# bliunlpr/Robust_e2e_gan

Hardware: NVIDIA B200
Metric: utterances/sec (joint step fwd/bwd) (higher is better)
Workload: dtype fp32

## Files before the change

### robust_e2e_gan_b200/csrc/attloc_loop.cu

```cuda
#include <math_constants.h>

#include "attloc_common.cuh"
#include "tc_common.cuh"

namespace re2e {
namespace {

#ifdef RE2E_ATT_DEBUG
__device__ long long g_loop_dbg[2][16 * 512];
#define LOOP_DBG_DECL                                                  \
  __shared__ long long dbg_acc[16];                                    \
  if (threadIdx.x == 0)                                                \
    for (int i_ = 0; i_ < 16; ++i_) dbg_acc[i_] = 0;                   \
  long long dbg_last = clock64()
#define LOOP_MARK(slot)                                              \
  do {                                                               \
    if (threadIdx.x == 0) {                                          \
      const long long t_ = clock64();                                \
      dbg_acc[slot] += t_ - dbg_last;                                \
      dbg_last = t_;                                                 \
    }                                                                \
  } while (0)
#define LOOP_DBG_FLUSH(which)                                                                   \
  do {                                                                                          \
    if (threadIdx.x == 0)                                                                       \
      for (int i_ = 0; i_ < 16; ++i_) g_loop_dbg[which][blockIdx.x * 16 + i_] = dbg_acc[i_];    \
  } while (0)
#else
#define LOOP_DBG_DECL
#define LOOP_MARK(slot)
#define LOOP_DBG_FLUSH(which)
#endif

__device__ __forceinline__ void cp_async4(void *dst_smem, const void *src_gmem) {
  asm volatile("cp.async.ca.shared.global [%0], [%1], 4;" ::"r"(smem_u32(dst_smem)), "l"(src_gmem) : "memory");
}
__device__ __forceinline__ void cp_async_commit() { asm volatile("cp.async.commit_group;" ::: "memory"); }
__device__ __forceinline__ void cp_async_wait_all() { asm volatile("cp.async.wait_group 0;" ::: "memory"); }

__device__ __forceinline__ void warp_reduce10(float (&v)[10], int lane) {
  {
    const bool up = lane & 16;
#pragma unroll
    for (int i = 0; i < 5; ++i) {
      const float send = up ? v[i] : v[i + 5], keep = up ? v[i + 5] : v[i];
      v[i] = keep + __shfl_xor_sync(0xffffffffu, send, 16);
    }
  }
  {
    const bool up = lane & 8;
#pragma unroll
    for (int i = 0; i < 2; ++i) {
      const float send = up ? v[i] : v[i + 3], keep = up ? v[i + 3] : v[i];
// ... 11 lines not shown
    const bool up = lane & 2;
    const float send = up ? v[0] : v[2], keep = up ? v[2] : v[0];
    v[0] = keep + __shfl_xor_sync(0xffffffffu, send, 2);
  }
  v[0] += __shfl_xor_sync(0xffffffffu, v[0], 1);
}

constexpr int kLP = 8;
constexpr int kLW = 2 * kLP;
constexpr int kLT = kLW * 32;
constexpr int kLMaxCL = 8;
constexpr int kKG = 12;

struct LoopGeom {
  int tloc_max, App, CKp, Thp, Dp;
  int col_enc, ncols;
};

struct LoopFwdParams {
  const float *pre, *enc, *dec_proj, *att_init, *W_att, *W_conv, *gvec, *gvec_b;
  float scaling;
  float *c_all, *w_all, *conv_all;
  int S, B, Th, D, A, C, K;
  LoopGeom g;
};

struct LoopBwdParams {
  const float *pre, *enc, *dec_proj, *att_init, *w_all, *conv_all, *dc_all, *dw_all, *W_att, *W_conv, *gvec;
  float scaling;
  float *d_pre, *d_decproj, *acc_slots;
  int slot_stride;
  int S, B, Th, D, A, C, K;
  LoopGeom g;
};

template <int APL, int CP, int DPL>
__global__ void __launch_bounds__(kLT, 1) attloc_loop_fwd_kernel(const LoopFwdParams p) {
  constexpr int NT = kLT;
  constexpr int WP = CP + 1;
  constexpr int CPP = (CP + 3) & ~3;
  extern __shared__ __align__(128) unsigned char smraw[];
  const LoopGeom g = p.g;
  const int C = CP == 10 ? 10 : p.C;
  const int Th = p.Th, D = p.D, A = p.A, K = p.K, S = p.S, B = p.B, filts = (p.K - 1) / 2;
  const int tid = threadIdx.x, lane = tid & 31, warp = tid >> 5, half = warp & 1, pair = warp >> 1;
  const int CL = (int)cluster_nctarank(), rank = (int)cluster_ctarank();
  const int b = blockIdx.x / CL;
  const int t0 = min(Th, rank * g.tloc_max), t1 = min(Th, t0 + g.tloc_max), tloc = t1 - t0;
  const int nch = (tloc + kLP - 1) / kLP;
  const int Dp = g.Dp, Dh = (D + 1) / 2;

  uint64_t *full = reinterpret_cast<uint64_t *>(smraw);
  uint64_t *xbar = full + 1;
  uint64_t *tbar = xbar + 2;
  float *tile = reinterpret_cast<float *>(smraw + 128);
  float *app = tile + (size_t)g.tloc_max * (A + D);
  float *wc_s = app + g.App;
  float *watt_s = wc_s + g.CKp;
  float *convp = watt_s + A * WP;
  float *conv_s = convp + round4(kKQ * g.tloc_max * CP);
  float *e_all = conv_s + g.tloc_max * CPP;
  float *epart = e_all + 2 * g.Thp;
  float *cred = epart + round4(2 * g.tloc_max);
  float *cbuf = cred + kLP * Dp;

  const uint32_t xbytes = (uint32_t)Th * 4u + (rank == 0 ? (uint32_t)CL * (uint32_t)D * 4u : 0u);
  if (tid == 0) {
    mbar_init(full, 1);
    mbar_init(&xbar[0], 1);
    mbar_init(&xbar[1], 1);
    mbar_init(tbar, 1);
    mbar_fence_init();
    mbar_expect_tx(&xbar[0], xbytes);
    mbar_expect_tx(&xbar[1], xbytes);
    if (rank == 0) mbar_expect_tx(tbar, (uint32_t)CL * (uint32_t)D * 4u);
  }
  cluster_arrive_relaxed();
  float gv[APL];
#pragma unroll
  for (int j = 0; j < APL; ++j) gv[j] = __ldg(p.gvec + half * (A / 2) + lane + 32 * j);
  const float gb = __ldg(p.gvec_b);
  for (int i = tid; i < C * K; i += NT) wc_s[i] = __ldg(p.W_conv + i);
  for (int i = tid; i < A * C; i += NT) { const int a = i / C; watt_s[a * WP + (i - a * C)] = __ldg(p.W_att + i); }
  pdl_wait();
  if (tid == 0 && tloc > 0) {
    mbar_expect_tx(full, (uint32_t)tloc * (uint32_t)(A + D) * 4u);
    bulk_g2s(tile, p.pre + ((size_t)b * Th + t0) * A, (uint32_t)tloc * A * 4u, full);
    bulk_g2s(tile + (size_t)g.tloc_max * A, p.enc + ((size_t)b * Th + t0) * D, (uint32_t)tloc * D * 4u, full);
  }
  for (int i = tid; i < g.App; i += NT) {
    const int t = i - filts;
    app[i] = (t >= 0 && t < Th) ? __ldg(p.att_init + (size_t)b * Th + t) : 0.0f;
  }
  __syncthreads();
  constexpr int APH = (APL + 1) / 2;
  float2 WattP[APH][CP];
#pragma unroll
  for (int jp = 0; jp < APH; ++jp) {
    const int a0 = half * (A / 2) + lane + 32 * (2 * jp), a1 = a0 + 32;
#pragma unroll
    for (int c = 0; c < CP; ++c)
      WattP[jp][c] = make_float2(c < C ? watt_s[a0 * WP + c] : 0.0f, (c < C && 2 * jp + 1 < APL) ? watt_s[a1 * WP + c] : 0.0f);
  }
  uint32_t dmask = 0;
#pragma unroll
  for (int j = 0; j < DPL; ++j)
    if (lane + 32 * j < Dh && half * Dh + lane + 32 * j < D) dmask |= 1u << j;
  const int aoff = half * (A / 2) + lane;
  cluster_wait();
  if (tloc > 0) mbar_wait(full, 0);
  LOOP_DBG_DECL;
  LOOP_MARK(0);

  for (int s = 0; s < S; ++s) {
    const uint32_t par = (uint32_t)s & 1u, ph = ((uint32_t)s >> 1) & 1u;
    float *e_cur = e_all + par * g.Thp;
    float *cb = cbuf + par * kLMaxCL * Dp;
    float dp[APL];
#pragma unroll
    for (int j = 0; j < APL; ++j) dp[j] = __ldg(p.dec_proj + ((size_t)s * B + b) * A + aoff + 32 * j);

    {
      const int ntg = (tloc + kTG - 1) / kTG;
      const int Kq = (K + kKQ - 1) / kKQ;
      const int nitems = ntg * C * kKQ;
      for (int item = tid; item < nitems; item += NT) {
        const int tg = item % ntg, rest = item / ntg, c = rest % C, kq = rest / C;
        const int k0 = kq * Kq, k1 = min(K, k0 + Kq);
        const float *wr = wc_s + c * K;
        const float *ar = app + t0 + kTG * tg;
        float a0 = 0.f, a1 = 0.f, a2 = 0.f, a3 = 0.f, a4 = 0.f;
        float x0 = ar[k0], x1 = ar[k0 + 1], x2 = ar[k0 + 2], x3 = ar[k0 + 3];
// ... 16 lines not shown
    __syncthreads();
    LOOP_MARK(1);
    for (int i = tid; i < tloc * CPP; i += NT) {
      const int tl = i / CPP, c = i - tl * CPP;
      float v = 0.0f;
      if (c < C) {
#pragma unroll
        for (int kq = 0; kq < kKQ; ++kq) v += convp[((size_t)kq * g.tloc_max + tl) * CP + c];
        if (p.conv_all) p.conv_all[(((size_t)s * B + b) * Th + t0 + tl) * C + c] = v;
      }
      conv_s[i] = v;
    }
    __syncthreads();
    LOOP_MARK(2);

    float acc[DPL];
#pragma unroll
    for (int j = 0; j < DPL; ++j) acc[j] = 0.0f;
#pragma unroll 2
    for (int q = 0; q < nch; ++q) {
      const int tl = kLP * q + pair;
      if (tl < tloc) {
        const float *cvp = conv_s + tl * CPP;
        float cv[CPP];
#pragma unroll
        for (int c4 = 0; c4 < CPP; c4 += 4) {
          const float4 t4 = *reinterpret_cast<const float4 *>(cvp + c4);
          cv[c4] = t4.x; cv[c4 + 1] = t4.y; cv[c4 + 2] = t4.z; cv[c4 + 3] = t4.w;
        }
        const float *row = tile + (size_t)tl * A + aoff;
        const float pw = app[filts + t0 + tl];
        const float *er = tile + (size_t)g.tloc_max * A + (size_t)tl * D + half * Dh + lane;
        float part = 0.0f;
#pragma unroll
        for (int jp = 0; jp < APH; ++jp) {
          const bool two = 2 * jp + 1 < APL;
          float2 u = make_float2(dp[2 * jp] + row[64 * jp], two ? dp[2 * jp + 1] + row[64 * jp + 32] : 0.0f);
#pragma unroll
          for (int c = 0; c < CP; ++c) u = __ffma2_rn(WattP[jp][c], make_float2(cv[c], cv[c]), u);
          part = fmaf(gv[2 * jp], tanh_ex2(u.x), part);
          if (two) part = fmaf(gv[2 * jp + 1], tanh_ex2(u.y), part);
        }
#pragma unroll
        for (int j = 0; j < DPL; ++j)
          if (dmask & (1u << j)) acc[j] = fmaf(pw, er[32 * j], acc[j]);
        part = warp_sum(part);
        if (lane == 0) epart[2 * tl + half] = part;
      }
    }
#pragma unroll
    for (int j = 0; j < DPL; ++j)
      if (dmask & (1u << j)) cred[pair * Dp + half * Dh + lane + 32 * j] = acc[j];
    LOOP_MARK(3);
    __syncthreads();
    LOOP_MARK(4);

    for (int d = tid; d < D; d += NT) {
      float sum = 0.0f;
#pragma unroll
      for (int pr = 0; pr < kLP; ++pr) sum += cred[pr * Dp + d];
      st_async_f32(dsmem_addr(cb + rank * Dp + d, 0u), s > 0 ? sum : 0.0f, dsmem_addr(&xbar[par], 0u));
    }
    for (int i = tid; i < tloc * CL; i += NT) {
      const int r = i / tloc, tl = i - r * tloc;
      const float e = p.scaling * ((epart[2 * tl] + epart[2 * tl + 1]) + gb);
      st_async_f32(dsmem_addr(e_cur + t0 + tl, (uint32_t)r), e, dsmem_addr(&xbar[par], (uint32_t)r));
    }
    LOOP_MARK(5);
    mbar_wait(&xbar[par], ph);
    LOOP_MARK(6);
    float M = -CUDART_INF_F;
    for (int t = lane; t < Th; t += 32) M = fmaxf(M, e_cur[t]);
    M = warp_max(M);
    float Ssum = 0.0f;
    for (int t = lane; t < Th; t += 32) Ssum += __expf(e_cur[t] - M);
    Ssum = warp_sum(Ssum);
    const float inv = 1.0f / Ssum;
    for (int t = tid; t < Th; t += NT) {
      const float w = __expf(e_cur[t] - M) * inv;
      app[filts + t] = w;
      if (t >= t0 && t < t1) p.w_all[((size_t)s * B + b) * Th + t] = w;
    }
    if (rank == 0 && s > 0) {
      for (int d = tid; d < D; d += NT) {
        float sum = 0.0f;
        for (int r = 0; r < CL; ++r) sum += cb[r * Dp + d];
        p.c_all[((size_t)(s - 1) * B + b) * D + d] = sum;
      }
    }
    if (tid == 0) mbar_expect_tx(&xbar[par], xbytes);
    __syncthreads();
    LOOP_MARK(7);
  }
  {
    float acc[DPL];
#pragma unroll
    for (int j = 0; j < DPL; ++j) acc[j] = 0.0f;
    for (int q = 0; q < nch; ++q) {
      const int tl = kLP * q + pair;
      if (tl < tloc) {
        const float pw = app[filts + t0 + tl];
        const float *er = tile + (size_t)g.tloc_max * A + (size_t)tl * D + half * Dh + lane;
#pragma unroll
        for (int j = 0; j < DPL; ++j)
          if (dmask & (1u << j)) acc[j] = fmaf(pw, er[32 * j], acc[j]);
      }
    }
#pragma unroll
    for (int j = 0; j < DPL; ++j)
      if (dmask & (1u << j)) cred[pair * Dp + half * Dh + lane + 32 * j] = acc[j];
    __syncthreads();
    float *cb = cbuf + ((uint32_t)S & 1u) * kLMaxCL * Dp;
    for (int d = tid; d < D; d += NT) {
      float sum = 0.0f;
#pragma unroll
      for (int pr = 0; pr < kLP; ++pr) sum += cred[pr * Dp + d];
      st_async_f32(dsmem_addr(cb + rank * Dp + d, 0u), sum, dsmem_addr(tbar, 0u));
    }
    if (rank == 0) {
      mbar_wait(tbar, 0);
      for (int d = tid; d < D; d += NT) {
        float sum = 0.0f;
        for (int r = 0; r < CL; ++r) sum += cb[r * Dp + d];
        p.c_all[((size_t)(S - 1) * B + b) * D + d] = sum;
      }
    }
  }
  LOOP_DBG_FLUSH(0);
}

template <int N>
__device__ __forceinline__ void tmem_ldn(uint32_t taddr, float *v);
template <>
__device__ __forceinline__ void tmem_ldn<1>(uint32_t taddr, float *v) {
  uint32_t r0;
  asm volatile("tcgen05.ld.sync.aligned.32x32b.x1.b32 {%0}, [%1];" : "=r"(r0) : "r"(taddr));
  v[0] = __uint_as_float(r0);
}
template <>
__device__ __forceinline__ void tmem_ldn<2>(uint32_t taddr, float *v) {
  uint32_t r0, r1;
  asm volatile("tcgen05.ld.sync.aligned.32x32b.x2.b32 {%0, %1}, [%2];" : "=r"(r0), "=r"(r1) : "r"(taddr));
// ... 47 lines not shown
template <int N>
__device__ __forceinline__ void tmem_load(uint32_t taddr, float *v) {
  if constexpr (N >= 8) { tmem_ldn<8>(taddr, v); if constexpr (N > 8) tmem_load<N - 8>(taddr + 8, v + 8); }
  else if constexpr (N >= 4) { tmem_ldn<4>(taddr, v); if constexpr (N > 4) tmem_load<N - 4>(taddr + 4, v + 4); }
  else if constexpr (N >= 2) { tmem_ldn<2>(taddr, v); if constexpr (N > 2) tmem_load<N - 2>(taddr + 2, v + 2); }
  else { tmem_ldn<1>(taddr, v); }
}
template <int N>
__device__ __forceinline__ void tmem_store(uint32_t taddr, const float *v) {
  if constexpr (N >= 8) { tmem_stn<8>(taddr, v); if constexpr (N > 8) tmem_store<N - 8>(taddr + 8, v + 8); }
  else if constexpr (N >= 4) { tmem_stn<4>(taddr, v); if constexpr (N > 4) tmem_store<N - 4>(taddr + 4, v + 4); }
  else if constexpr (N >= 2) { tmem_stn<2>(taddr, v); if constexpr (N > 2) tmem_store<N - 2>(taddr + 2, v + 2); }
  else { tmem_stn<1>(taddr, v); }
}

template <int APL, int CP, int DPL2>
__global__ void __launch_bounds__(kLT, 1) attloc_loop_bwd_kernel(const LoopBwdParams p) {
  constexpr int NT = kLT;
  constexpr int WP = CP + 1;
  constexpr int CPP = (CP + 3) & ~3;
  constexpr int CH2 = (CP + 1) / 2;
  extern __shared__ __align__(128) unsigned char smraw[];
  const LoopGeom g = p.g;
  const int C = CP == 10 ? 10 : p.C;
  const int Th = p.Th, D = p.D, A = p.A, K = p.K, S = p.S, B = p.B, filts = (p.K - 1) / 2;
  const int tid = threadIdx.x, lane = tid & 31, warp = tid >> 5, half = warp & 1, pair = warp >> 1;
  const int CL = (int)cluster_nctarank(), rank = (int)cluster_ctarank();
  const int b = blockIdx.x / CL;
  const int t0 = min(Th, rank * g.tloc_max), t1 = min(Th, t0 + g.tloc_max), tloc = t1 - t0;
  const int nchx = (tloc + kLP - 1) / kLP;
  const int nche = (tloc + kLW - 1) / kLW;
  const int nchx_max = (g.tloc_max + kLP - 1) / kLP, nche_max = (g.tloc_max + kLW - 1) / kLW;

  uint64_t *done_x = reinterpret_cast<uint64_t *>(smraw);
  uint64_t *xbar1 = done_x + 1;
  uint64_t *xbar2 = xbar1 + 2;
  uint32_t *tmem_slot = reinterpret_cast<uint32_t *>(xbar2 + 2);
  float *xs = reinterpret_cast<float *>(smraw + 128);
  float *dcvT = xs + (size_t)g.tloc_max * A;
  float *app = dcvT + 2 * CP * g.App;
  float *wc_s = app + g.App;
  float *conv_s = wc_s + g.CKp;
  float *w_s = conv_s + g.tloc_max * CPP;
  float *dwt_s = w_s + round4(g.tloc_max);
  float *de_s = dwt_s + round4(g.tloc_max);
  float *dwn_s = de_s + round4(g.tloc_max);
  float *dcv_p = dwn_s + round4(g.tloc_max);
  float *ddp_w = dcv_p + 2 * g.tloc_max * 16;
  float *scr = ddp_w + kLW * (A / 2);
  float *ddp_x = scr + max(A * WP, round4(kKQ * CP * g.tloc_max));
  float *xch = ddp_x + 2 * kLMaxCL * A;
  float *slot = p.acc_slots + (size_t)blockIdx.x * p.slot_stride;

  const uint32_t x1bytes = (uint32_t)CL * 4u;
  const uint32_t x2bytes = (uint32_t)Th * (uint32_t)C * 4u + (rank == 0 ? (uint32_t)CL * (uint32_t)A * 4u : 0u);
  if (tid == 0) {
    mbar_init(done_x, kLW);
    for (int i = 0; i < 2; ++i) { mbar_init(&xbar1[i], 1); mbar_init(&xbar2[i], 1); }
    mbar_fence_init();
    for (int i = 0; i < 2; ++i) { mbar_expect_tx(&xbar1[i], x1bytes); mbar_expect_tx(&xbar2[i], x2bytes); }
  }
  cluster_arrive_relaxed();
  if (warp == 0) tmem_alloc(tmem_slot, 512);
  float gv[APL];
#pragma unroll
  for (int j = 0; j < APL; ++j) gv[j] = __ldg(p.gvec + half * (A / 2) + lane + 32 * j);
  for (int i = tid; i < C * K; i += NT) wc_s[i] = __ldg(p.W_conv + i);
  for (int i = tid; i < A * C; i += NT) { const int a = i / C; scr[a * WP + (i - a * C)] = __ldg(p.W_att + i); }
  {
    const int padn = g.App - Th;
    for (int i = tid; i < 2 * CP * padn; i += NT) {
      const int c = i / padn, o = i - c * padn;
      dcvT[c * g.App + (o < filts ? o : Th + o)] = 0.0f;
    }
    for (int i = tid; i < g.tloc_max * CPP; i += NT) conv_s[i] = 0.0f;
    for (int i = tid; i < round4(g.tloc_max); i += NT) dwn_s[i] = 0.0f;
  }
  tc_fence_before();
  __syncthreads();
  tc_fence_after();
  const uint32_t tbase = *tmem_slot + ((uint32_t)(32 * (warp & 3)) << 16);
  const uint32_t tcol_pre = tbase + (uint32_t)((warp >> 2) * nchx_max * APL);
  const uint32_t tcol_enc = tbase + (uint32_t)(g.col_enc + (warp >> 2) * nche_max * DPL2);
  float2 WattC[APL][CH2];
#pragma unroll
  for (int j = 0; j < APL; ++j) {
    const int a = half * (A / 2) + lane + 32 * j;
#pragma unroll
    for (int c2 = 0; c2 < CH2; ++c2)
      WattC[j][c2] = make_float2(2 * c2 < C ? scr[a * WP + 2 * c2] : 0.0f, 2 * c2 + 1 < C ? scr[a * WP + 2 * c2 + 1] : 0.0f);
  }
  const int aoff = half * (A / 2) + lane;
  pdl_wait();
  for (int q = 0; q < nchx; ++q) {
    const int tl = kLP * q + pair;
    float v[APL];
#pragma unroll
    for (int j = 0; j < APL; ++j) v[j] = tl < tloc ? __ldg(p.pre + ((size_t)b * Th + t0 + tl) * A + aoff + 32 * j) : 0.0f;
    tmem_store<APL>(tcol_pre + (uint32_t)(q * APL), v);
  }
  for (int q = 0; q < nche; ++q) {
    const int tl = kLW * q + warp;
    float v[DPL2];
#pragma unroll
    for (int j = 0; j < DPL2; ++j)
      v[j] = (tl < tloc && lane + 32 * j < D) ? __ldg(p.enc + ((size_t)b * Th + t0 + tl) * D + lane + 32 * j) : 0.0f;
    tmem_store<DPL2>(tcol_enc + (uint32_t)(q * DPL2), v);
  }
  tmem_wait_st();
  __syncthreads();
  cluster_wait();

  float pacc[kKG];
#pragma unroll
  for (int i = 0; i < kKG; ++i) pacc[i] = 0.0f;
  float dgv[APL];
#pragma unroll
  for (int j = 0; j < APL; ++j) dgv[j] = 0.0f;
  float dgb = 0.0f;
  const int nkg = (K + kKG - 1) / kKG;
  const bool conv_thread = tid >= A && tid - A < C * nkg;
  const int cw_c = conv_thread ? (tid - A) / nkg : 0, cw_kb = conv_thread ? ((tid - A) % nkg) * kKG : 0;
  LOOP_DBG_DECL;
  LOOP_MARK(0);

  for (int it = 0; it < S; ++it) {
    const int s = S - 1 - it;
    const uint32_t par = (uint32_t)it & 1u, ph = ((uint32_t)it >> 1) & 1u;
    float *dcv_cur = dcvT + par * CP * g.App;
    float *ddpx = ddp_x + par * kLMaxCL * A;
    float *xc = xch + par * kLMaxCL;
    const size_t sb = (size_t)s * B + b;
    float dcr[DPL2];
#pragma unroll
    for (int j = 0; j < DPL2; ++j) dcr[j] = (p.dc_all && lane + 32 * j < D) ? __ldg(p.dc_all + sb * D + lane + 32 * j) : 0.0f;
    float dp[APL];
#pragma unroll
    for (int j = 0; j < APL; ++j) dp[j] = __ldg(p.dec_proj + sb * A + aoff + 32 * j);
    for (int i = tid; i < tloc; i += NT) {
      w_s[i] = __ldg(p.w_all + sb * Th + t0 + i);
      dwt_s[i] = dwn_s[i] + (p.dw_all ? __ldg(p.dw_all + sb * Th + t0 + i) : 0.0f);
    }
    for (int i = tid; i < tloc * C; i += NT) {
      const int tl = i / C;
      conv_s[tl * CPP + (i - tl * C)] = __ldg(p.conv_all + (sb * Th + t0) * C + i);
    }
    {
      const float *prev = s == 0 ? p.att_init + (size_t)b * Th : p.w_all + (sb - B) * Th;
      for (int i = tid; i < g.App; i += NT) {
        const int t = i - filts;
        app[i] = (t >= 0 && t < Th) ? __ldg(prev + t) : 0.0f;
      }
    }
    __syncthreads();
    LOOP_MARK(1);

    for (int q = 0; q < nche; ++q) {
      const int tl = kLW * q + warp;
      float ev[DPL2];
      tmem_load<DPL2>(tcol_enc + (uint32_t)(q * DPL2), ev);
      tmem_wait_ld();
      float dot = 0.0f;
#pragma unroll
      for (int j = 0; j < DPL2; ++j) dot = fmaf(dcr[j], ev[j], dot);
      dot = warp_sum(dot);
      if (lane == 0 && tl < tloc) dwt_s[tl] += dot;
    }
    __syncthreads();
    LOOP_MARK(2);
    if (warp == 0) {
      float s1 = 0.0f;
      for (int tl = lane; tl < tloc; tl += 32) s1 = fmaf(w_s[tl], dwt_s[tl], s1);
      s1 = warp_sum(s1);
      if (lane < CL) st_async_f32(dsmem_addr(xc + rank, (uint32_t)lane), s1, dsmem_addr(&xbar1[par], (uint32_t)lane));
    }
    mbar_wait(&xbar1[par], ph);
    float Stot = 0.0f;
    for (int r = 0; r < CL; ++r) Stot += xc[r];
    for (int tl = tid; tl < tloc; tl += NT) de_s[tl] = p.scaling * w_s[tl] * (dwt_s[tl] - Stot);
    if (tid == 0) {
      mbar_expect_tx(&xbar1[par], x1bytes);
// ... 87 lines not shown
    for (int j = 0; j < APL; ++j) ddp_w[warp * (A / 2) + lane + 32 * j] = ddp[j];
    __syncthreads();
    LOOP_MARK(5);

    for (int item = tid; item < tloc * C; item += NT) {
      const int c = item / tloc, tl = item - c * tloc;
      const float v = dcv_p[tl * 16 + c] + dcv_p[(g.tloc_max + tl) * 16 + c];
      for (int r = 0; r < CL; ++r)
        st_async_f32(dsmem_addr(dcv_cur + c * g.App + filts + t0 + tl, (uint32_t)r), v, dsmem_addr(&xbar2[par], (uint32_t)r));
    }
    for (int a = tid; a < A; a += NT) {
      const int h = a >= A / 2 ? 1 : 0, ai = a - h * (A / 2);
      float sd = 0.0f;
#pragma unroll
      for (int pr = 0; pr < kLP; ++pr) sd += ddp_w[(2 * pr + h) * (A / 2) + ai];
      st_async_f32(dsmem_addr(ddpx + rank * A + a, 0u), sd, dsmem_addr(&xbar2[par], 0u));
    }
    if (warp == kLW - 1) {
      float s2 = 0.0f;
      for (int tl = lane; tl < tloc; tl += 32) s2 += de_s[tl];
      dgb += warp_sum(s2);
    }
    LOOP_MARK(6);
    if (tid < A) {
#pragma unroll 5
      for (int tl = 0; tl < tloc; ++tl) {
        const float dt = xs[(size_t)tl * A + tid];
#pragma unroll
        for (int c4 = 0; c4 < CPP; c4 += 4) {
          const float4 t4 = *reinterpret_cast<const float4 *>(conv_s + tl * CPP + c4);
          if (c4 < CP) pacc[c4] = fmaf(dt, t4.x, pacc[c4]);
// ... 8 lines not shown
#pragma unroll
      for (int i = 0; i < kKG - 1; ++i) x[i] = ar[t0 + i];
#pragma unroll 12
      for (int tl = 0; tl < tloc; ++tl) {
        x[kKG - 1] = ar[t0 + tl + kKG - 1];
        const float dv = dcv_p[tl * 16 + cw_c] + dcv_p[(g.tloc_max + tl) * 16 + cw_c];
#pragma unroll
        for (int i = 0; i < kKG; ++i) pacc[i] = fmaf(dv, x[i], pacc[i]);
#pragma unroll
        for (int i = 0; i < kKG - 1; ++i) x[i] = x[i + 1];
      }
    }
    LOOP_MARK(7);
    mbar_wait(&xbar2[par], ph);
    LOOP_MARK(8);
    if (rank == 0) {
      for (int a = tid; a < A; a += NT) {
        float sd = 0.0f;
        for (int r = 0; r < CL; ++r) sd += ddpx[r * A + a];
        p.d_decproj[sb * A + a] = sd;
      }
    }
    if (s > 0) {
      const int nsg = (tloc + kTG - 1) / kTG;
      const int Kq = (K + kKQ - 1) / kKQ;
      const int nitems = nsg * C * kKQ;
      for (int item = tid; item < nitems; item += NT) {
        const int sg = item % nsg, rest = item / nsg, c = rest % C, kq = rest / C;
        const int k0 = kq * Kq, k1 = min(K, k0 + Kq);
        const float *wr = wc_s + c * K;
        const float *dr = dcv_cur + c * g.App + (t0 + kTG * sg) + 2 * filts;
        float a0 = 0.f, a1 = 0.f, a2 = 0.f, a3 = 0.f, a4 = 0.f;
        float x1 = dr[1 - k0], x2 = dr[2 - k0], x3 = dr[3 - k0], x4 = dr[4 - k0];
#pragma unroll 5
        for (int k = k0; k < k1; ++k) {
          const float x0 = dr[-k], wv = wr[k];
// ... 63 lines not shown
inline int pick_cl(int B, int Th) {
  const int sms = num_sms();
  int CL = 1;
  while (CL < kLMaxCL && B * CL * 2 <= sms) CL *= 2;
  while (CL > 1 && (Th + CL - 1) / CL < kLP) CL /= 2;
  return CL;
}

inline void loop_geom_common(int Th, int D, int C, int K, int CL, LoopGeom &g) {
  const int filts = (K - 1) / 2;
  g.tloc_max = (Th + CL - 1) / CL;
  g.App = round4(Th + 2 * filts + 8);
  g.CKp = round4(C * K);
  g.Thp = round4(Th);
  g.Dp = round4(D);
  g.col_enc = 0;
  g.ncols = 0;
}

inline bool loop_geom_fwd(int B, int Th, int D, int A, int C, int K, int CP, int &CL, LoopGeom &g, size_t &smem) {
  CL = pick_cl(B, Th);
  const int CPP = round4(CP);
  for (;;) {
    loop_geom_common(Th, D, C, K, CL, g);
    const size_t floats = (size_t)g.tloc_max * (A + D) + g.App + g.CKp + (size_t)A * (CP + 1) +
                          round4(kKQ * g.tloc_max * CP) + (size_t)g.tloc_max * CPP + 2 * (size_t)g.Thp +
                          round4(g.tloc_max) + round4(2 * g.tloc_max) + 2 * kLW + (size_t)kLP * g.Dp +
                          2 * (size_t)kLMaxCL * g.Dp + 4 * kLMaxCL;
    smem = 128 + sizeof(float) * floats;
    if (smem <= 226 * 1024) return true;
    if (CL >= kLMaxCL || B * CL * 2 > num_sms()) return false;
    CL *= 2;
  }
}

inline bool loop_geom_bwd(int B, int Th, int D, int A, int C, int K, int CP, int dpl2, int &CL, LoopGeom &g,
                          size_t &smem) {
  CL = pick_cl(B, Th);
  const int CPP = round4(CP);
  const int nkg = (K + kKG - 1) / kKG;
  if (A + C * nkg > kLT) return false;
  for (;;) {
    loop_geom_common(Th, D, C, K, CL, g);
    const int nchx_max = (g.tloc_max + kLP - 1) / kLP, nche_max = (g.tloc_max + kLW - 1) / kLW;
    g.col_enc = 4 * nchx_max * (A / 64);
    g.ncols = g.col_enc + 4 * nche_max * dpl2;
    const size_t scr = (size_t)A * (CP + 1) > (size_t)round4(kKQ * CP * g.tloc_max) ? (size_t)A * (CP + 1)
                                                                                   : (size_t)round4(kKQ * CP * g.tloc_max);
    const size_t floats = (size_t)g.tloc_max * A + 2 * (size_t)CP * g.App + g.App + g.CKp + (size_t)g.tloc_max * CPP +
                          4 * (size_t)round4(g.tloc_max) + 2 * (size_t)g.tloc_max * 16 + (size_t)kLW * (A / 2) + scr +
                          2 * (size_t)kLMaxCL * A + 2 * kLMaxCL;
    smem = 128 + sizeof(float) * floats;
    if (smem <= 226 * 1024 && g.ncols <= 512) return true;
    if (CL >= kLMaxCL || B * CL * 2 > num_sms()) return false;
    CL *= 2;
  }
}

template <typename Kern, typename Params>
int launch_loop(Kern kern, const Params &prm, int B, int CL, size_t smem, cudaStream_t st) {
  int rc0 = ensure_smem(reinterpret_cast<const void *>(kern), smem);
  if (rc0 != RE2E_OK) return rc0;
  cudaLaunchConfig_t cfg{};
  cfg.gridDim = dim3((unsigned)(B * CL));
  cfg.blockDim = dim3((unsigned)kLT);
  cfg.dynamicSmemBytes = smem;
  cfg.stream = st;
  cudaLaunchAttribute attr[2];
// ... 10 lines not shown
  return e == cudaSuccess ? RE2E_OK : (int)e;
}

#define LOOP_DISPATCH(NAME, APLV, CPV, ...)                                             \
  switch (APLV) {                                                                       \
    case 1: rc = (CPV) == 10 ? NAME<1, 10> __VA_ARGS__ : NAME<1, 16> __VA_ARGS__; break; \
    case 2: rc = (CPV) == 10 ? NAME<2, 10> __VA_ARGS__ : NAME<2, 16> __VA_ARGS__; break; \
    case 4: rc = (CPV) == 10 ? NAME<4, 10> __VA_ARGS__ : NAME<4, 16> __VA_ARGS__; break; \
    case 5: rc = (CPV) == 10 ? NAME<5, 10> __VA_ARGS__ : NAME<5, 16> __VA_ARGS__; break; \
    case 8: rc = (CPV) == 10 ? NAME<8, 10> __VA_ARGS__ : NAME<8, 16> __VA_ARGS__; break; \
    default: rc = RE2E_E_UNSUPPORTED;                                                   \
  }

template <int APL, int CP>
int run_loop_fwd(const LoopFwdParams &prm, int CL, size_t smem, cudaStream_t st) {
  if (prm.D == prm.A) return launch_loop(attloc_loop_fwd_kernel<APL, CP, APL>, prm, prm.B, CL, smem, st);
  return launch_loop(attloc_loop_fwd_kernel<APL, CP, 8>, prm, prm.B, CL, smem, st);
}
template <int APL, int CP>
int run_loop_bwd(const LoopBwdParams &prm, int CL, size_t smem, cudaStream_t st) {
  if (prm.D == prm.A) return launch_loop(attloc_loop_bwd_kernel<APL, CP, 2 * APL>, prm, prm.B, CL, smem, st);
  return launch_loop(attloc_loop_bwd_kernel<APL, CP, 16>, prm, prm.B, CL, smem, st);
}

}
}

using namespace re2e;

#ifdef RE2E_ATT_DEBUG
extern "C" int re2e_loop_debug_read(long long *host_out, int which) {
  cudaDeviceSynchronize();
  return (int)cudaMemcpyFromSymbol(host_out, g_loop_dbg, sizeof(long long) * 16 * 512, sizeof(long long) * 16 * 512 * which);
}
#endif

extern "C" int re2e_attloc_loop_supported(int S, int B, int Th, int D, int A, int C, int K) {
  int rc = loop_check_dims(S, B, Th, D, A, C, K);
  if (rc != RE2E_OK) return 0;
  const int CP = C == 10 ? 10 : 16;
  int CLf, CLb;
  size_t smem;
  LoopGeom g;
  if (!loop_geom_fwd(B, Th, D, A, C, K, CP, CLf, g, smem)) return 0;
  if (!loop_geom_bwd(B, Th, D, A, C, K, CP, D == A ? 2 * (A / 64) : 16, CLb, g, smem)) return 0;
  return 1;
}

extern "C" int re2e_attloc_loop_slots(int S, int B, int Th, int D, int A, int C, int K) {
  int rc = loop_check_dims(S, B, Th, D, A, C, K);
  if (rc != RE2E_OK) return rc;
  int CL;
  size_t smem;
  LoopGeom g;
  if (!loop_geom_bwd(B, Th, D, A, C, K, C == 10 ? 10 : 16, D == A ? 2 * (A / 64) : 16, CL, g, smem))
    return RE2E_E_UNSUPPORTED;
  return B * CL;
}

extern "C" int re2e_attloc_loop_fwd(const float *pre, const float *enc_h, const float *dec_proj,
                                    const float *att_init, const float *W_att, const float *W_conv,
                                    const float *gvec, const float *gvec_b, float scaling, float *c_all,
                                    float *w_all, float *conv_all, int S, int B, int Th, int D, int A, int C,
                                    int K, void *stream) {
  RE2E_CHECK_ARG(pre && enc_h && dec_proj && att_init && W_att && W_conv && gvec && gvec_b && c_all && w_all);
  int rc = loop_check_dims(S, B, Th, D, A, C, K);
  if (rc != RE2E_OK) return rc;
  RE2E_CHECK_ARG(aligned16(pre) && aligned16(enc_h));
  const int CP = C == 10 ? 10 : 16;
  LoopFwdParams prm;
  prm.pre = pre; prm.enc = enc_h; prm.dec_proj = dec_proj; prm.att_init = att_init; prm.W_att = W_att;
  prm.W_conv = W_conv; prm.gvec = gvec; prm.gvec_b = gvec_b; prm.scaling = scaling; prm.c_all = c_all;
  prm.w_all = w_all; prm.conv_all = conv_all;
  prm.S = S; prm.B = B; prm.Th = Th; prm.D = D; prm.A = A; prm.C = C; prm.K = K;
  int CL;
  size_t smem;
  if (!loop_geom_fwd(B, Th, D, A, C, K, CP, CL, prm.g, smem)) return RE2E_E_UNSUPPORTED;
  LOOP_DISPATCH(run_loop_fwd, A / 64, CP, (prm, CL, smem, static_cast<cudaStream_t>(stream)));
  return rc;
}

extern "C" int re2e_attloc_loop_bwd(const float *pre, const float *enc_h, const float *dec_proj,
                                    const float *att_init, const float *w_all, const float *conv_all,
                                    const float *dc_all, const float *dw_all, const float *W_att,
                                    const float *W_conv, const float *gvec, float scaling, float *d_pre,
                                    float *d_decproj, float *acc_slots, int n_slots, int S, int B, int Th, int D,
                                    int A, int C, int K, void *stream) {
  RE2E_CHECK_ARG(pre && enc_h && dec_proj && att_init && w_all && conv_all && W_att && W_conv && gvec);
  RE2E_CHECK_ARG(d_pre && d_decproj && acc_slots);
  int rc = loop_check_dims(S, B, Th, D, A, C, K);
  if (rc != RE2E_OK) return rc;
  RE2E_CHECK_ARG(aligned16(d_pre));
  const int CP = C == 10 ? 10 : 16;
  LoopBwdParams prm;
  prm.pre = pre; prm.enc = enc_h; prm.dec_proj = dec_proj; prm.att_init = att_init; prm.w_all = w_all;
  prm.conv_all = conv_all; prm.dc_all = dc_all; prm.dw_all = dw_all; prm.W_att = W_att; prm.W_conv = W_conv;
  prm.gvec = gvec; prm.scaling = scaling; prm.d_pre = d_pre; prm.d_decproj = d_decproj; prm.acc_slots = acc_slots;
  prm.slot_stride = (int)re2e_attloc_acc_floats(A, C, K);
  prm.S = S; prm.B = B; prm.Th = Th; prm.D = D; prm.A = A; prm.C = C; prm.K = K;
  int CL;
  size_t smem;
  if (!loop_geom_bwd(B, Th, D, A, C, K, CP, D == A ? 2 * (A / 64) : 16, CL, prm.g, smem)) return RE2E_E_UNSUPPORTED;
  if (n_slots < B * CL) return RE2E_E_WORKSPACE;
  LOOP_DISPATCH(run_loop_bwd, A / 64, CP, (prm, CL, smem, static_cast<cudaStream_t>(stream)));
  return rc;
}
```

Measured before the change: 24860.

## Batch context accumulation out of the attention step loop into chunked GEMM passes

In the forward kernel, the per-step context vector (weights times encoder rows) is taken out of the serial recurrence. It is now computed after the loop in chunks of SC steps as a small register-tiled GEMM with paired FMAs, and cluster partials are reduced over DSMEM with the work split across ranks. The backward kernel likewise precomputes dc·enc dot products for chunks of steps instead of per-step TMEM-held encoder loads, and it distributes the d_decproj reduction across all cluster ranks instead of rank 0. This shortens the latency-critical sequential path, at the cost of extra shared memory, re-reading w_all from global, and additional cluster syncs.

```diff
diff --git a/robust_e2e_gan_b200/csrc/attloc_loop.cu b/robust_e2e_gan_b200/csrc/attloc_loop.cu
--- a/robust_e2e_gan_b200/csrc/attloc_loop.cu
+++ b/robust_e2e_gan_b200/csrc/attloc_loop.cu
@@ -32,11 +32,12 @@
 #define LOOP_DBG_FLUSH(which)
 #endif
 
-__device__ __forceinline__ void cp_async4(void *dst_smem, const void *src_gmem) {
-  asm volatile("cp.async.ca.shared.global [%0], [%1], 4;" ::"r"(smem_u32(dst_smem)), "l"(src_gmem) : "memory");
-}
-__device__ __forceinline__ void cp_async_commit() { asm volatile("cp.async.commit_group;" ::: "memory"); }
-__device__ __forceinline__ void cp_async_wait_all() { asm volatile("cp.async.wait_group 0;" ::: "memory"); }
+__device__ __forceinline__ float4 dsmem_ld4(uint32_t addr) {
+  float4 v;
+  asm volatile("ld.shared::cluster.v4.f32 {%0, %1, %2, %3}, [%4];" : "=f"(v.x), "=f"(v.y), "=f"(v.z), "=f"(v.w) : "r"(addr)
+               : "memory");
+  return v;
+}
 
 __device__ __forceinline__ void warp_reduce10(float (&v)[10], int lane) {
   {
@@ -78,7 +79,8 @@
 
 struct LoopGeom {
   int tloc_max, App, CKp, Thp, Dp;
-  int col_enc, ncols;
+  int sc;
+  int ncols;
 };
 
 struct LoopFwdParams {
@@ -98,7 +100,7 @@
   LoopGeom g;
 };
 
-template <int APL, int CP, int DPL>
+template <int APL, int CP>
 __global__ void __launch_bounds__(kLT, 1) attloc_loop_fwd_kernel(const LoopFwdParams p) {
   constexpr int NT = kLT;
   constexpr int WP = CP + 1;
@@ -112,32 +114,30 @@
   const int b = blockIdx.x / CL;
   const int t0 = min(Th, rank * g.tloc_max), t1 = min(Th, t0 + g.tloc_max), tloc = t1 - t0;
   const int nch = (tloc + kLP - 1) / kLP;
-  const int Dp = g.Dp, Dh = (D + 1) / 2;
+  const int Dp = g.Dp;
 
   uint64_t *full = reinterpret_cast<uint64_t *>(smraw);
   uint64_t *xbar = full + 1;
-  uint64_t *tbar = xbar + 2;
-  float *tile = reinterpret_cast<float *>(smraw + 128);
-  float *app = tile + (size_t)g.tloc_max * (A + D);
+  float *enc_s = reinterpret_cast<float *>(smraw + 128);
+  float *tile = enc_s + (size_t)g.tloc_max * D;
+  float *app = tile + (size_t)g.tloc_max * A;
   float *wc_s = app + g.App;
   float *watt_s = wc_s + g.CKp;
   float *convp = watt_s + A * WP;
   float *conv_s = convp + round4(kKQ * g.tloc_max * CP);
   float *e_all = conv_s + g.tloc_max * CPP;
   float *epart = e_all + 2 * g.Thp;
-  float *cred = epart + round4(2 * g.tloc_max);
-  float *cbuf = cred + kLP * Dp;
-
-  const uint32_t xbytes = (uint32_t)Th * 4u + (rank == 0 ? (uint32_t)CL * (uint32_t)D * 4u : 0u);
+  float *pctx = tile;
+  float *wst = pctx + (size_t)g.sc * Dp;
+
+  const uint32_t xbytes = (uint32_t)Th * 4u;
   if (tid == 0) {
     mbar_init(full, 1);
     mbar_init(&xbar[0], 1);
     mbar_init(&xbar[1], 1);
-    mbar_init(tbar, 1);
     mbar_fence_init();
     mbar_expect_tx(&xbar[0], xbytes);
     mbar_expect_tx(&xbar[1], xbytes);
-    if (rank == 0) mbar_expect_tx(tbar, (uint32_t)CL * (uint32_t)D * 4u);
   }
   cluster_arrive_relaxed();
   float gv[APL];
@@ -150,7 +150,7 @@
   if (tid == 0 && tloc > 0) {
     mbar_expect_tx(full, (uint32_t)tloc * (uint32_t)(A + D) * 4u);
     bulk_g2s(tile, p.pre + ((size_t)b * Th + t0) * A, (uint32_t)tloc * A * 4u, full);
-    bulk_g2s(tile + (size_t)g.tloc_max * A, p.enc + ((size_t)b * Th + t0) * D, (uint32_t)tloc * D * 4u, full);
+    bulk_g2s(enc_s, p.enc + ((size_t)b * Th + t0) * D, (uint32_t)tloc * D * 4u, full);
   }
   for (int i = tid; i < g.App; i += NT) {
     const int t = i - filts;
@@ -166,10 +166,6 @@
     for (int c = 0; c < CP; ++c)
       WattP[jp][c] = make_float2(c < C ? watt_s[a0 * WP + c] : 0.0f, (c < C && 2 * jp + 1 < APL) ? watt_s[a1 * WP + c] : 0.0f);
   }
-  uint32_t dmask = 0;
-#pragma unroll
-  for (int j = 0; j < DPL; ++j)
-    if (lane + 32 * j < Dh && half * Dh + lane + 32 * j < D) dmask |= 1u << j;
   const int aoff = half * (A / 2) + lane;
   cluster_wait();
   if (tloc > 0) mbar_wait(full, 0);
@@ -179,7 +175,6 @@
   for (int s = 0; s < S; ++s) {
     const uint32_t par = (uint32_t)s & 1u, ph = ((uint32_t)s >> 1) & 1u;
     float *e_cur = e_all + par * g.Thp;
-    float *cb = cbuf + par * kLMaxCL * Dp;
     float dp[APL];
 #pragma unroll
     for (int j = 0; j < APL; ++j) dp[j] = __ldg(p.dec_proj + ((size_t)s * B + b) * A + aoff + 32 * j);
@@ -226,9 +221,6 @@
     __syncthreads();
     LOOP_MARK(2);
 
-    float acc[DPL];
-#pragma unroll
-    for (int j = 0; j < DPL; ++j) acc[j] = 0.0f;
 #pragma unroll 2
     for (int q = 0; q < nch; ++q) {
       const int tl = kLP * q + pair;
@@ -241,8 +233,6 @@
           cv[c4] = t4.x; cv[c4 + 1] = t4.y; cv[c4 + 2] = t4.z; cv[c4 + 3] = t4.w;
         }
         const float *row = tile + (size_t)tl * A + aoff;
-        const float pw = app[filts + t0 + tl];
-        const float *er = tile + (size_t)g.tloc_max * A + (size_t)tl * D + half * Dh + lane;
         float part = 0.0f;
 #pragma unroll
         for (int jp = 0; jp < APH; ++jp) {
@@ -253,26 +243,14 @@
           part = fmaf(gv[2 * jp], tanh_ex2(u.x), part);
           if (two) part = fmaf(gv[2 * jp + 1], tanh_ex2(u.y), part);
         }
-#pragma unroll
-        for (int j = 0; j < DPL; ++j)
-          if (dmask & (1u << j)) acc[j] = fmaf(pw, er[32 * j], acc[j]);
         part = warp_sum(part);
         if (lane == 0) epart[2 * tl + half] = part;
       }
     }
-#pragma unroll
-    for (int j = 0; j < DPL; ++j)
-      if (dmask & (1u << j)) cred[pair * Dp + half * Dh + lane + 32 * j] = acc[j];
     LOOP_MARK(3);
     __syncthreads();
     LOOP_MARK(4);
 
-    for (int d = tid; d < D; d += NT) {
-      float sum = 0.0f;
-#pragma unroll
-      for (int pr = 0; pr < kLP; ++pr) sum += cred[pr * Dp + d];
-      st_async_f32(dsmem_addr(cb + rank * Dp + d, 0u), s > 0 ? sum : 0.0f, dsmem_addr(&xbar[par], 0u));
-    }
     for (int i = tid; i < tloc * CL; i += NT) {
       const int r = i / tloc, tl = i - r * tloc;
       const float e = p.scaling * ((epart[2 * tl] + epart[2 * tl + 1]) + gb);
@@ -293,51 +271,70 @@
       app[filts + t] = w;
       if (t >= t0 && t < t1) p.w_all[((size_t)s * B + b) * Th + t] = w;
     }
-    if (rank == 0 && s > 0) {
-      for (int d = tid; d < D; d += NT) {
-        float sum = 0.0f;
-        for (int r = 0; r < CL; ++r) sum += cb[r * Dp + d];
-        p.c_all[((size_t)(s - 1) * B + b) * D + d] = sum;
-      }
-    }
     if (tid == 0) mbar_expect_tx(&xbar[par], xbytes);
     __syncthreads();
     LOOP_MARK(7);
   }
-  {
-    float acc[DPL];
-#pragma unroll
-    for (int j = 0; j < DPL; ++j) acc[j] = 0.0f;
-    for (int q = 0; q < nch; ++q) {
-      const int tl = kLP * q + pair;
-      if (tl < tloc) {
-        const float pw = app[filts + t0 + tl];
-        const float *er = tile + (size_t)g.tloc_max * A + (size_t)tl * D + half * Dh + lane;
-#pragma unroll
-        for (int j = 0; j < DPL; ++j)
-          if (dmask & (1u << j)) acc[j] = fmaf(pw, er[32 * j], acc[j]);
-      }
-    }
-#pragma unroll
-    for (int j = 0; j < DPL; ++j)
-      if (dmask & (1u << j)) cred[pair * Dp + half * Dh + lane + 32 * j] = acc[j];
+
+  const int SC = g.sc, DQ = D / 4;
+  for (int s0 = 0; s0 < S; s0 += SC) {
+    const int ns = min(SC, S - s0);
+    for (int i = tid; i < tloc * SC; i += NT) {
+      const int sl = i / tloc, tl = i - sl * tloc;
+      wst[tl * SC + sl] = sl < ns ? p.w_all[((size_t)(s0 + sl) * B + b) * Th + t0 + tl] : 0.0f;
+    }
     __syncthreads();
-    float *cb = cbuf + ((uint32_t)S & 1u) * kLMaxCL * Dp;
-    for (int d = tid; d < D; d += NT) {
-      float sum = 0.0f;
-#pragma unroll
-      for (int pr = 0; pr < kLP; ++pr) sum += cred[pr * Dp + d];
-      st_async_f32(dsmem_addr(cb + rank * Dp + d, 0u), sum, dsmem_addr(tbar, 0u));
-    }
-    if (rank == 0) {
-      mbar_wait(tbar, 0);
-      for (int d = tid; d < D; d += NT) {
-        float sum = 0.0f;
-        for (int r = 0; r < CL; ++r) sum += cb[r * Dp + d];
-        p.c_all[((size_t)(S - 1) * B + b) * D + d] = sum;
-      }
-    }
-  }
+    for (int item = tid; item < (SC / 4) * DQ; item += NT) {
+      const int sg = item / DQ, dq = item - sg * DQ;
+      const float *er = enc_s + 4 * dq;
+      const float *wr = wst + 4 * sg;
+      float tot[4][4];
+#pragma unroll
+      for (int i = 0; i < 4; ++i)
+#pragma unroll
+        for (int c = 0; c < 4; ++c) tot[i][c] = 0.0f;
+#pragma unroll 1
+      for (int pr = 0; pr < kLP; ++pr) {
+        float2 acc[4][2];
+#pragma unroll
+        for (int i = 0; i < 4; ++i) acc[i][0] = acc[i][1] = make_float2(0.0f, 0.0f);
+#pragma unroll 2
+        for (int tl = pr; tl < tloc; tl += kLP) {
+          const float4 e = *reinterpret_cast<const float4 *>(er + (size_t)tl * D);
+          const float4 w4 = *reinterpret_cast<const float4 *>(wr + tl * SC);
+          const float wv[4] = {w4.x, w4.y, w4.z, w4.w};
+#pragma unroll
+          for (int i = 0; i < 4; ++i) {
+            acc[i][0] = __ffma2_rn(make_float2(wv[i], wv[i]), make_float2(e.x, e.y), acc[i][0]);
+            acc[i][1] = __ffma2_rn(make_float2(wv[i], wv[i]), make_float2(e.z, e.w), acc[i][1]);
+          }
+        }
+#pragma unroll
+        for (int i = 0; i < 4; ++i) {
+          tot[i][0] += acc[i][0].x; tot[i][1] += acc[i][0].y; tot[i][2] += acc[i][1].x; tot[i][3] += acc[i][1].y;
+        }
+      }
+#pragma unroll
+      for (int i = 0; i < 4; ++i)
+        *reinterpret_cast<float4 *>(pctx + (size_t)(4 * sg + i) * Dp + 4 * dq) =
+            make_float4(tot[i][0], tot[i][1], tot[i][2], tot[i][3]);
+    }
+    cluster_sync_all();
+    const int nq = ns * DQ, lo = nq * rank / CL, hi = nq * (rank + 1) / CL;
+    for (int i = lo + tid; i < hi; i += NT) {
+      const int sl = i / DQ, dq = i - sl * DQ;
+      const float *src = pctx + (size_t)sl * Dp + 4 * dq;
+      float4 sum = make_float4(0.0f, 0.0f, 0.0f, 0.0f);
+      for (int r = 0; r < CL; ++r) {
+        const float4 v = dsmem_ld4(dsmem_addr(src, (uint32_t)r));
+        sum.x += v.x; sum.y += v.y; sum.z += v.z; sum.w += v.w;
+      }
+      float *dst = p.c_all + ((size_t)(s0 + sl) * B + b) * D + 4 * dq;
+      dst[0] = sum.x; dst[1] = sum.y; dst[2] = sum.z; dst[3] = sum.w;
+    }
+    cluster_sync_all();
+  }
+  LOOP_MARK(8);
   LOOP_DBG_FLUSH(0);
 }
 
@@ -415,7 +412,7 @@
   else { tmem_stn<1>(taddr, v); }
 }
 
-template <int APL, int CP, int DPL2>
+template <int APL, int CP>
 __global__ void __launch_bounds__(kLT, 1) attloc_loop_bwd_kernel(const LoopBwdParams p) {
   constexpr int NT = kLT;
   constexpr int WP = CP + 1;
@@ -430,8 +427,8 @@
   const int b = blockIdx.x / CL;
   const int t0 = min(Th, rank * g.tloc_max), t1 = min(Th, t0 + g.tloc_max), tloc = t1 - t0;
   const int nchx = (tloc + kLP - 1) / kLP;
-  const int nche = (tloc + kLW - 1) / kLW;
-  const int nchx_max = (g.tloc_max + kLP - 1) / kLP, nche_max = (g.tloc_max + kLW - 1) / kLW;
+  const int nchx_max = (g.tloc_max + kLP - 1) / kLP;
+  const int tlp = round4(g.tloc_max);
 
   uint64_t *done_x = reinterpret_cast<uint64_t *>(smraw);
   uint64_t *xbar1 = done_x + 1;
@@ -450,11 +447,13 @@
   float *ddp_w = dcv_p + 2 * g.tloc_max * 16;
   float *scr = ddp_w + kLW * (A / 2);
   float *ddp_x = scr + max(A * WP, round4(kKQ * CP * g.tloc_max));
-  float *xch = ddp_x + 2 * kLMaxCL * A;
+  float *xch = ddp_x + 2 * A;
+  float *dwc_s = xch + 2 * kLMaxCL;
   float *slot = p.acc_slots + (size_t)blockIdx.x * p.slot_stride;
 
   const uint32_t x1bytes = (uint32_t)CL * 4u;
-  const uint32_t x2bytes = (uint32_t)Th * (uint32_t)C * 4u + (rank == 0 ? (uint32_t)CL * (uint32_t)A * 4u : 0u);
+  const uint32_t x2bytes = (uint32_t)Th * (uint32_t)C * 4u + (uint32_t)A * 4u;
+  const int Ar = A / CL;
   if (tid == 0) {
     mbar_init(done_x, kLW);
     for (int i = 0; i < 2; ++i) { mbar_init(&xbar1[i], 1); mbar_init(&xbar2[i], 1); }
@@ -482,7 +481,6 @@
   tc_fence_after();
   const uint32_t tbase = *tmem_slot + ((uint32_t)(32 * (warp & 3)) << 16);
   const uint32_t tcol_pre = tbase + (uint32_t)((warp >> 2) * nchx_max * APL);
-  const uint32_t tcol_enc = tbase + (uint32_t)(g.col_enc + (warp >> 2) * nche_max * DPL2);
   float2 WattC[APL][CH2];
 #pragma unroll
   for (int j = 0; j < APL; ++j) {
@@ -499,14 +497,6 @@
 #pragma unroll
     for (int j = 0; j < APL; ++j) v[j] = tl < tloc ? __ldg(p.pre + ((size_t)b * Th + t0 + tl) * A + aoff + 32 * j) : 0.0f;
     tmem_store<APL>(tcol_pre + (uint32_t)(q * APL), v);
-  }
-  for (int q = 0; q < nche; ++q) {
-    const int tl = kLW * q + warp;
-    float v[DPL2];
-#pragma unroll
-    for (int j = 0; j < DPL2; ++j)
-      v[j] = (tl < tloc && lane + 32 * j < D) ? __ldg(p.enc + ((size_t)b * Th + t0 + tl) * D + lane + 32 * j) : 0.0f;
-    tmem_store<DPL2>(tcol_enc + (uint32_t)(q * DPL2), v);
   }
   tmem_wait_st();
   __syncthreads();
@@ -529,18 +519,49 @@
     const int s = S - 1 - it;
     const uint32_t par = (uint32_t)it & 1u, ph = ((uint32_t)it >> 1) & 1u;
     float *dcv_cur = dcvT + par * CP * g.App;
-    float *ddpx = ddp_x + par * kLMaxCL * A;
+    float *ddpx = ddp_x + par * A;
     float *xc = xch + par * kLMaxCL;
     const size_t sb = (size_t)s * B + b;
-    float dcr[DPL2];
-#pragma unroll
-    for (int j = 0; j < DPL2; ++j) dcr[j] = (p.dc_all && lane + 32 * j < D) ? __ldg(p.dc_all + sb * D + lane + 32 * j) : 0.0f;
+    if (p.dc_all && it % g.sc == 0) {
+      if (tid == 0 && it > 0) bulk_wait<0>();
+      __syncthreads();
+      const int scr_n = max(A * WP, round4(kKQ * CP * g.tloc_max));
+      float *dcs = g.tloc_max * A >= scr_n ? xs : scr;
+      const int ns = min(g.sc, S - it), G = max(g.tloc_max * A, scr_n) / g.Dp;
+      for (int p0 = 0; p0 < ns; p0 += G) {
+        const int ng = min(G, ns - p0);
+        for (int i = tid; i < ng * D; i += NT) {
+          const int sl = i / D, d = i - sl * D;
+          dcs[sl * g.Dp + d] = __ldg(p.dc_all + ((size_t)(S - 1 - it - p0 - sl) * B + b) * D + d);
+        }
+        __syncthreads();
+        for (int tl = warp; tl < tloc; tl += kLW) {
+          float ev[16];
+#pragma unroll
+          for (int j = 0; j < 16; ++j)
+            ev[j] = lane + 32 * j < D ? __ldg(p.enc + ((size_t)b * Th + t0 + tl) * D + lane + 32 * j) : 0.0f;
+#pragma unroll 2
+          for (int sl = 0; sl < ng; ++sl) {
+            const float *dr = dcs + sl * g.Dp + lane;
+            float dot = 0.0f;
+#pragma unroll
+            for (int j = 0; j < 16; ++j)
+              if (lane + 32 * j < D) dot = fmaf(dr[32 * j], ev[j], dot);
+            dot = warp_sum(dot);
+            if (lane == 0) dwc_s[(p0 + sl) * tlp + tl] = dot;
+          }
+        }
+        __syncthreads();
+      }
+    }
+    LOOP_MARK(1);
+    const float *dwc = dwc_s + (it % g.sc) * tlp;
     float dp[APL];
 #pragma unroll
     for (int j = 0; j < APL; ++j) dp[j] = __ldg(p.dec_proj + sb * A + aoff + 32 * j);
     for (int i = tid; i < tloc; i += NT) {
       w_s[i] = __ldg(p.w_all + sb * Th + t0 + i);
-      dwt_s[i] = dwn_s[i] + (p.dw_all ? __ldg(p.dw_all + sb * Th + t0 + i) : 0.0f);
+      dwt_s[i] = dwn_s[i] + (p.dw_all ? __ldg(p.dw_all + sb * Th + t0 + i) : 0.0f) + (p.dc_all ? dwc[i] : 0.0f);
     }
     for (int i = tid; i < tloc * C; i += NT) {
       const int tl = i / C;
@@ -552,20 +573,6 @@
         const int t = i - filts;
         app[i] = (t >= 0 && t < Th) ? __ldg(prev + t) : 0.0f;
       }
-    }
-    __syncthreads();
-    LOOP_MARK(1);
-
-    for (int q = 0; q < nche; ++q) {
-      const int tl = kLW * q + warp;
-      float ev[DPL2];
-      tmem_load<DPL2>(tcol_enc + (uint32_t)(q * DPL2), ev);
-      tmem_wait_ld();
-      float dot = 0.0f;
-#pragma unroll
-      for (int j = 0; j < DPL2; ++j) dot = fmaf(dcr[j], ev[j], dot);
-      dot = warp_sum(dot);
-      if (lane == 0 && tl < tloc) dwt_s[tl] += dot;
     }
     __syncthreads();
     LOOP_MARK(2);
@@ -683,7 +690,8 @@
       float sd = 0.0f;
 #pragma unroll
       for (int pr = 0; pr < kLP; ++pr) sd += ddp_w[(2 * pr + h) * (A / 2) + ai];
-      st_async_f32(dsmem_addr(ddpx + rank * A + a, 0u), sd, dsmem_addr(&xbar2[par], 0u));
+      const int o = a / Ar;
+      st_async_f32(dsmem_addr(ddpx + rank * Ar + (a - o * Ar), (uint32_t)o), sd, dsmem_addr(&xbar2[par], (uint32_t)o));
     }
     if (warp == kLW - 1) {
       float s2 = 0.0f;
@@ -722,12 +730,10 @@
     LOOP_MARK(7);
     mbar_wait(&xbar2[par], ph);
     LOOP_MARK(8);
-    if (rank == 0) {
-      for (int a = tid; a < A; a += NT) {
-        float sd = 0.0f;
-        for (int r = 0; r < CL; ++r) sd += ddpx[r * A + a];
-        p.d_decproj[sb * A + a] = sd;
-      }
+    for (int i = tid; i < Ar; i += NT) {
+      float sd = 0.0f;
+      for (int r = 0; r < CL; ++r) sd += ddpx[r * Ar + i];
+      p.d_decproj[sb * A + rank * Ar + i] = sd;
     }
     if (s > 0) {
       const int nsg = (tloc + kTG - 1) / kTG;
@@ -821,44 +827,52 @@
   g.CKp = round4(C * K);
   g.Thp = round4(Th);
   g.Dp = round4(D);
-  g.col_enc = 0;
+  g.sc = 0;
   g.ncols = 0;
 }
 
-inline bool loop_geom_fwd(int B, int Th, int D, int A, int C, int K, int CP, int &CL, LoopGeom &g, size_t &smem) {
+inline bool loop_geom_fwd(int S, int B, int Th, int D, int A, int C, int K, int CP, int &CL, LoopGeom &g,
+                          size_t &smem) {
   CL = pick_cl(B, Th);
   const int CPP = round4(CP);
   for (;;) {
     loop_geom_common(Th, D, C, K, CL, g);
-    const size_t floats = (size_t)g.tloc_max * (A + D) + g.App + g.CKp + (size_t)A * (CP + 1) +
-                          round4(kKQ * g.tloc_max * CP) + (size_t)g.tloc_max * CPP + 2 * (size_t)g.Thp +
-                          round4(g.tloc_max) + round4(2 * g.tloc_max) + 2 * kLW + (size_t)kLP * g.Dp +
-                          2 * (size_t)kLMaxCL * g.Dp + 4 * kLMaxCL;
-    smem = 128 + sizeof(float) * floats;
+    size_t after_enc = (size_t)g.tloc_max * A + g.App + g.CKp + (size_t)A * (CP + 1) + round4(kKQ * g.tloc_max * CP) +
+                       (size_t)g.tloc_max * CPP + 2 * (size_t)g.Thp + round4(2 * g.tloc_max);
+    const size_t per_step = (size_t)g.Dp + g.tloc_max;
+    const size_t fit = (after_enc / per_step) & ~(size_t)3;
+    g.sc = (int)std::max<size_t>(4, std::min<size_t>(fit, (size_t)round4(S)));
+    after_enc = std::max(after_enc, (size_t)g.sc * per_step);
+    smem = 128 + sizeof(float) * ((size_t)g.tloc_max * D + after_enc);
     if (smem <= 226 * 1024) return true;
     if (CL >= kLMaxCL || B * CL * 2 > num_sms()) return false;
     CL *= 2;
   }
 }
 
-inline bool loop_geom_bwd(int B, int Th, int D, int A, int C, int K, int CP, int dpl2, int &CL, LoopGeom &g,
+inline bool loop_geom_bwd(int S, int B, int Th, int D, int A, int C, int K, int CP, int &CL, LoopGeom &g,
                           size_t &smem) {
   CL = pick_cl(B, Th);
   const int CPP = round4(CP);
   const int nkg = (K + kKG - 1) / kKG;
   if (A + C * nkg > kLT) return false;
+  constexpr size_t kMax = 226 * 1024;
   for (;;) {
     loop_geom_common(Th, D, C, K, CL, g);
-    const int nchx_max = (g.tloc_max + kLP - 1) / kLP, nche_max = (g.tloc_max + kLW - 1) / kLW;
-    g.col_enc = 4 * nchx_max * (A / 64);
-    g.ncols = g.col_enc + 4 * nche_max * dpl2;
+    const int nchx_max = (g.tloc_max + kLP - 1) / kLP;
+    g.ncols = 4 * nchx_max * (A / 64);
     const size_t scr = (size_t)A * (CP + 1) > (size_t)round4(kKQ * CP * g.tloc_max) ? (size_t)A * (CP + 1)
                                                                                    : (size_t)round4(kKQ * CP * g.tloc_max);
     const size_t floats = (size_t)g.tloc_max * A + 2 * (size_t)CP * g.App + g.App + g.CKp + (size_t)g.tloc_max * CPP +
                           4 * (size_t)round4(g.tloc_max) + 2 * (size_t)g.tloc_max * 16 + (size_t)kLW * (A / 2) + scr +
-                          2 * (size_t)kLMaxCL * A + 2 * kLMaxCL;
+                          2 * (size_t)A + 2 * kLMaxCL;
     smem = 128 + sizeof(float) * floats;
-    if (smem <= 226 * 1024 && g.ncols <= 512) return true;
+    const size_t per_step = sizeof(float) * round4(g.tloc_max);
+    if (smem + per_step <= kMax && g.ncols <= 512) {
+      g.sc = (int)std::min<size_t>((size_t)S, (kMax - smem) / per_step);
+      smem += (size_t)g.sc * per_step;
+      return true;
+    }
     if (CL >= kLMaxCL || B * CL * 2 > num_sms()) return false;
     CL *= 2;
   }
@@ -899,13 +913,11 @@
 
 template <int APL, int CP>
 int run_loop_fwd(const LoopFwdParams &prm, int CL, size_t smem, cudaStream_t st) {
-  if (prm.D == prm.A) return launch_loop(attloc_loop_fwd_kernel<APL, CP, APL>, prm, prm.B, CL, smem, st);
-  return launch_loop(attloc_loop_fwd_kernel<APL, CP, 8>, prm, prm.B, CL, smem, st);
+  return launch_loop(attloc_loop_fwd_kernel<APL, CP>, prm, prm.B, CL, smem, st);
 }
 template <int APL, int CP>
 int run_loop_bwd(const LoopBwdParams &prm, int CL, size_t smem, cudaStream_t st) {
-  if (prm.D == prm.A) return launch_loop(attloc_loop_bwd_kernel<APL, CP, 2 * APL>, prm, prm.B, CL, smem, st);
-  return launch_loop(attloc_loop_bwd_kernel<APL, CP, 16>, prm, prm.B, CL, smem, st);
+  return launch_loop(attloc_loop_bwd_kernel<APL, CP>, prm, prm.B, CL, smem, st);
 }
 
 }
@@ -927,8 +939,8 @@
   int CLf, CLb;
   size_t smem;
   LoopGeom g;
-  if (!loop_geom_fwd(B, Th, D, A, C, K, CP, CLf, g, smem)) return 0;
-  if (!loop_geom_bwd(B, Th, D, A, C, K, CP, D == A ? 2 * (A / 64) : 16, CLb, g, smem)) return 0;
+  if (!loop_geom_fwd(S, B, Th, D, A, C, K, CP, CLf, g, smem)) return 0;
+  if (!loop_geom_bwd(S, B, Th, D, A, C, K, CP, CLb, g, smem)) return 0;
   return 1;
 }
 
@@ -938,8 +950,7 @@
   int CL;
   size_t smem;
   LoopGeom g;
-  if (!loop_geom_bwd(B, Th, D, A, C, K, C == 10 ? 10 : 16, D == A ? 2 * (A / 64) : 16, CL, g, smem))
-    return RE2E_E_UNSUPPORTED;
+  if (!loop_geom_bwd(S, B, Th, D, A, C, K, C == 10 ? 10 : 16, CL, g, smem)) return RE2E_E_UNSUPPORTED;
   return B * CL;
 }
 
@@ -960,7 +971,7 @@
   prm.S = S; prm.B = B; prm.Th = Th; prm.D = D; prm.A = A; prm.C = C; prm.K = K;
   int CL;
   size_t smem;
-  if (!loop_geom_fwd(B, Th, D, A, C, K, CP, CL, prm.g, smem)) return RE2E_E_UNSUPPORTED;
+  if (!loop_geom_fwd(S, B, Th, D, A, C, K, CP, CL, prm.g, smem)) return RE2E_E_UNSUPPORTED;
   LOOP_DISPATCH(run_loop_fwd, A / 64, CP, (prm, CL, smem, static_cast<cudaStream_t>(stream)));
   return rc;
 }
@@ -985,7 +996,7 @@
   prm.S = S; prm.B = B; prm.Th = Th; prm.D = D; prm.A = A; prm.C = C; prm.K = K;
   int CL;
   size_t smem;
-  if (!loop_geom_bwd(B, Th, D, A, C, K, CP, D == A ? 2 * (A / 64) : 16, CL, prm.g, smem)) return RE2E_E_UNSUPPORTED;
+  if (!loop_geom_bwd(S, B, Th, D, A, C, K, CP, CL, prm.g, smem)) return RE2E_E_UNSUPPORTED;
   if (n_slots < B * CL) return RE2E_E_WORKSPACE;
   LOOP_DISPATCH(run_loop_bwd, A / 64, CP, (prm, CL, smem, static_cast<cudaStream_t>(stream)));
   return rc;
```

Result: slower. 22860, median of 6 (-8.1%).
